# qiyunzhu/woltka

Hardware: AMD Instinct MI355X
Metric: alignment records/sec classified (higher is better)
Workload: dtype u8; 1 GPU; synthetic SAM text of 50M reads x <=16 hits (10.50 GB) resident in HBM, 2M-node taxonomy, ranks phylum,genus,species: device tokenizer per 64 MB block + one weighted histogram per sample (the kernels of `woltka classify`, host link left out); records_per_gpu=250034804, reads_per_gpu=50000000

## Files before the change

### woltka_amd/csrc/wk_dtok_fused.hpp

```cpp
#pragma once
#include "wk_dtok.hpp"
#include "wk_dtok_planes.hpp"
#include "wk_dtok_rounds.hpp"

namespace wk {

constexpr uint32_t kFzThreads = 512;
constexpr uint32_t kFzWaves = kFzThreads / kWave;
constexpr uint32_t kFzTile = 16384;
constexpr uint32_t kFzBack = 1024;
constexpr uint32_t kFzFwd = 3072;
constexpr uint32_t kFzWin = kFzTile + kFzBack + kFzFwd;
constexpr uint32_t kFzChunks = kFzWin / 16 + 1;
constexpr uint32_t kFzRounds = kFrMaxRounds;
static_assert(kFrChunks * 16u == kFzWin && kFrTailChunk + 1u == kFzChunks && kFrWaves == kFzWaves && kFrWave == kWave,
              "the dealing covers the window");
constexpr uint32_t kFzLines = 1024;
constexpr uint32_t kFzStreams = 4;
constexpr uint32_t kFzCap = 1024;
static_assert(kFzCap >= kFzLines, "a window's records fit an empty buffer");
static_assert(kFzWin + 32 < 65536, "window offsets fit 16 bits");
constexpr uint32_t kFzCarry = 256;
static_assert(kFzCarry + kFzLines <= kFpMaxLines && kFzThreads % kWave == 0, "a window's owned lines fit the planes, a wave's lines one word");

constexpr uint32_t kDtokSpill = 64;

struct FusedArgs {
    const unsigned char* text;
    uint32_t n;
    uint32_t open_end;
    uint32_t span;
    const struct DictSlot8* dict8;
    const uint4* names16;
    uint32_t dict_mask;
    const unsigned char* arena;
    uint2* unknown;
    uint32_t unknown_cap;
    DtokState* state;
    DtokState* host_state;
    const unsigned long long* backup_prev;
    unsigned long long* backup_next;
    uint32_t* host_seq;
    uint32_t seq;
    StreamSet streams;
    const int32_t* submap;
    uint32_t n_submap;
    uint32_t ablate;
};

static_assert(sizeof(DtokState) % 8 == 0, "the packed totals are aligned");
__device__ __forceinline__ unsigned long long* fz_totals(DtokState* state) { return reinterpret_cast<unsigned long long*>(state + 1); }

__global__ void dtok_fused_begin_kernel(unsigned long long* __restrict__ backup, const unsigned long long* __restrict__ cursor, DtokState* state) {
    if (threadIdx.x < (uint32_t)kMaxStreams) backup[threadIdx.x] = cursor[threadIdx.x];
    if (threadIdx.x == 0) {
        *state = DtokState{0u, 0u, 0ull, 0ull, 0ull, 0u, 0u};
        *fz_totals(state) = 0ull;
    }
}

template <int kCtrl, int kRowMask>
__device__ __forceinline__ uint32_t fz_dpp_add(uint32_t v) {
    return v + (uint32_t)__builtin_amdgcn_update_dpp(0, (int)v, kCtrl, kRowMask, 0xF, false);
}
__device__ __forceinline__ uint32_t fz_wave_scan(uint32_t v) {
    static_assert(kWave == 64, "four rows of sixteen lanes");
    v = fz_dpp_add<0x111, 0xF>(v);
    v = fz_dpp_add<0x112, 0xF>(v);
    v = fz_dpp_add<0x114, 0xF>(v);
    v = fz_dpp_add<0x118, 0xF>(v);
    v = fz_dpp_add<0x142, 0xA>(v);
    v = fz_dpp_add<0x143, 0xC>(v);
    return v;
}
__device__ __forceinline__ uint32_t fz_last_lane(uint32_t v) { return (uint32_t)__builtin_amdgcn_readlane((int)v, kWave - 1); }
__device__ __forceinline__ uint32_t fz_wave_sum(uint32_t v) { return fz_last_lane(fz_wave_scan(v)); }
__device__ __forceinline__ unsigned long long fz_first_lane64(unsigned long long v) {
    return ((unsigned long long)(uint32_t)__builtin_amdgcn_readfirstlane((int)(uint32_t)(v >> 32)) << 32) |
           (uint32_t)__builtin_amdgcn_readfirstlane((int)(uint32_t)v);
}

__device__ __forceinline__ uint4 fz_load_stream(const unsigned char* p) {
    typedef uint32_t u32x4 __attribute__((ext_vector_type(4)));
    const u32x4 v = __builtin_nontemporal_load(reinterpret_cast<const u32x4*>(p));
    return make_uint4(v.x, v.y, v.z, v.w);
}
__device__ __forceinline__ unsigned long long fz_load64(const unsigned char* p) {
    unsigned long long w;
    __builtin_memcpy(&w, p, 8);
    return w;
}
__device__ __forceinline__ uint32_t fz_load32(const unsigned char* p) {
    uint32_t w;
    __builtin_memcpy(&w, p, 4);
    return w;
}
__device__ __forceinline__ unsigned long long fz_eq_bytes(unsigned long long w, unsigned char c) {
    const unsigned long long x = w ^ (0x0101010101010101ull * c);
    return ~(((x & 0x7F7F7F7F7F7F7F7Full) + 0x7F7F7F7F7F7F7F7Full) | x | 0x7F7F7F7F7F7F7F7Full);
}
__device__ __forceinline__ uint32_t fz_marks32(uint32_t w, uint32_t c4) {
    const uint32_t x = w ^ c4;
    return ~(((x & 0x7F7F7F7Fu) + 0x7F7F7F7Fu) | x | 0x7F7F7F7Fu);
}
__device__ __forceinline__ unsigned long long fz_low_bytes(unsigned long long w, uint32_t k) {
    return k >= 8u ? w : (w & ((1ull << (8u * k)) - 1ull));
}

__device__ __forceinline__ unsigned long long fz_hash(const unsigned char* p, uint32_t n) {
    unsigned long long h = 0xcbf29ce484222325ull ^ ((unsigned long long)n * 0x9E3779B97F4A7C15ull);
    while (n >= 8u) {
        h = (h ^ fz_load64(p)) * 0x100000001b3ull;
        h ^= h >> 29;
        p += 8;
        n -= 8u;
    }
    const unsigned long long v = n ? fz_low_bytes(fz_load64(p), n) : 0ull;
    h = (h ^ v) * 0x100000001b3ull;
    h ^= h >> 32;
    h *= 0x9E3779B97F4A7C15ull;
    return h ^ (h >> 29);
}

__device__ __forceinline__ bool fz_same(const unsigned char* x, const unsigned char* y, uint32_t n) {
    while (n >= 8u) {
        if (fz_load64(x) != fz_load64(y)) return false;
        x += 8;
        y += 8;
        n -= 8u;
    }
    return n == 0u || fz_low_bytes(fz_load64(x) ^ fz_load64(y), n) == 0ull;
}

struct FzProbe {
    unsigned long long hv, n0, n1;
    uint32_t h;
    uint2 slot;
};
__device__ __forceinline__ FzProbe fz_probe_begin(const FusedArgs& a, const unsigned char* name, uint32_t rn) {
    FzProbe p;
    p.hv = fz_hash(name, rn);
    p.n0 = p.n1 = 0ull;
    if (rn <= 15u) {
        p.n0 = fz_low_bytes(fz_load64(name), rn);
        p.n1 = (rn > 8u ? fz_low_bytes(fz_load64(name + 8), rn - 8u) : 0ull) | ((unsigned long long)rn << 56);
    }
    p.h = (uint32_t)p.hv & a.dict_mask;
    p.slot = reinterpret_cast<const uint2*>(a.dict8)[p.h];
    return p;
}
__device__ __forceinline__ int32_t fz_probe_end(const FusedArgs& a, FzProbe p, const unsigned char* name, uint32_t rn, uint32_t abs_off) {
    for (;;) {
        const int32_t id = (int32_t)p.slot.y;
        if (id < 0) break;
        if (p.slot.x == (uint32_t)(p.hv >> 32)) {
            const uint4 nm = a.names16[id];
            const unsigned long long s0 = ((unsigned long long)nm.y << 32) | nm.x, s1 = ((unsigned long long)nm.w << 32) | nm.z;
            if (rn <= 15u) {
                if (s0 == p.n0 && s1 == p.n1) return id;
            } else if ((nm.w >> 24) == 0xFFu) {
                const unsigned char* full = a.arena + nm.x;
                if (fz_load32(full) == rn && fz_same(name, full + 4, rn)) return id;
            }
        }
        p.h = (p.h + 1u) & a.dict_mask;
        p.slot = reinterpret_cast<const uint2*>(a.dict8)[p.h];
    }
    const uint32_t at = atomicAdd(&a.state->n_unknown, 1u);
    if (at < a.unknown_cap)
        a.unknown[at] = make_uint2(abs_off, rn);
    else
        atomicOr(&a.state->flags, kDtokUnknownFull);
    return kLineUnknown;
}

__device__ bool fz_starts_run_slow(const unsigned char* __restrict__ text, uint32_t at, const unsigned char* q, uint32_t qn) {
    uint32_t pos = at;
    while (pos > 0u) {
        const uint32_t e = pos - 1u;
        uint32_t s = e;
        while (s > 0u && text[s - 1u] != '\n') --s;
        uint32_t tab[3], nt = 0;
        for (uint32_t p = s; p < e && nt < 3u; ++p)
            if (text[p] == '\t') tab[nt++] = p;
        if (nt == 3u && !(tab[2] - tab[1] == 2u && text[tab[1] + 1u] == '*')) {
            if (tab[0] - s != qn) return true;
            for (uint32_t k = 0; k < qn; ++k)
                if (text[s + k] != q[k]) return true;
            return false;
        }
        pos = s;
    }
    return true;
}

constexpr uint32_t kFiSubj = (1u << 23) - 1u;
constexpr uint32_t kFiMateShift = 24;
constexpr uint32_t kFiMapped = 1u << 26;
constexpr uint32_t kFiStart = 1u << 27;
constexpr uint32_t kFiExcl = 1u << 29;
constexpr uint32_t kFiDropped = 1u << 30;
constexpr uint32_t kFiRead = kFiMapped | (3u << kFiMateShift);
constexpr uint32_t kFiKey = kFiRead | kFiSubj;
constexpr uint32_t kFzPad = 8;

__device__ __forceinline__ uint32_t fz_octet(uint32_t z_lo, uint32_t z_hi) { return (((z_lo >> 7) | (z_hi >> 3)) * 0x00204081u >> 21) & 255u; }

__device__ __forceinline__ uint32_t fz_newlines16(uint4 v) {
    return fz_octet(fz_marks32(v.x, 0x0A0A0A0Au), fz_marks32(v.y, 0x0A0A0A0Au)) | (fz_octet(fz_marks32(v.z, 0x0A0A0A0Au), fz_marks32(v.w, 0x0A0A0A0Au)) << 8);
}

__device__ __forceinline__ uint32_t fz_tabs32(const unsigned char* p) {
    unsigned long long w[4];
#pragma unroll
    for (uint32_t i = 0; i < 4; ++i) w[i] = fz_load64(p + 8u * i);
    uint32_t m = 0;
#pragma unroll
    for (uint32_t i = 0; i < 4; ++i)
        m |= fz_octet(fz_marks32((uint32_t)w[i], 0x09090909u), fz_marks32((uint32_t)(w[i] >> 32), 0x09090909u)) << (8u * i);
    return m;
}

__global__ void __launch_bounds__(kFzThreads) __attribute__((amdgpu_waves_per_eu(6, 6))) dtok_fused_kernel(FusedArgs a) {
    __shared__ __attribute__((aligned(16))) unsigned char txt[kFzChunks * 16 + 32];
    __shared__ uint16_t ls[kFzLines + 2];
    __shared__ uint16_t f_qn[kFzLines], f_rb[kFzLines], f_rn[kFzLines];
    __shared__ __attribute__((aligned(16))) uint32_t info_[kFzPad + kFzCarry + kFzLines + kFzPad + 8];
    __shared__ uint32_t carry[kFzCarry];
    __shared__ unsigned long long planes[kFpPlanes][kFpWords];
    __shared__ uint32_t rbuf[kFzStreams][kFzCap];
    __shared__ unsigned long long fill_packed;
    static_assert(kFzStreams <= 4 && kFzCap + kFzThreads < 65536, "four 16-bit counts");
    __shared__ unsigned long long gbase[kFzStreams];
    __shared__ uint32_t wtot[kFzWaves];
    __shared__ unsigned long long gbase_out[kMaxStreams];
    __shared__ unsigned long long wg_totals;
    __shared__ uint32_t own[4];
    __shared__ uint32_t wg_flags;
    uint32_t* const info = info_ + kFzPad + kFzCarry;

    const uint32_t tid = threadIdx.x, lane = tid & (kWave - 1), wave = tid / kWave;
    const uint32_t wave_s = (uint32_t)__builtin_amdgcn_readfirstlane((int)wave);
    const uint32_t n_streams = a.streams.n_streams;
    const uint32_t ablate = a.ablate;
    const int32_t* const submap = a.submap;
    unsigned long long fill = 0ull;
    if (tid == 0) fill_packed = 0ull;
    if (tid < 4u) reinterpret_cast<uint32_t*>(txt + kFrTailChunk * 16u)[tid] = 0u;
    if (tid == 0) wg_flags = 0u;
    if (tid == 0) wg_totals = 0ull;
    uint32_t my_flags = 0, my_reads = 0, my_lines = 0;
    const uint32_t text_end = a.n + (a.open_end ? 1u : 0u);

    auto flush_all = [&](unsigned long long have, bool last) {
        __syncthreads();
        if (tid < n_streams) {
            const uint32_t cnt = (ablate & 64u) ? 0u : (uint32_t)(have >> (16u * tid)) & 0xFFFFu;
            unsigned long long base = 0ull;
            if (cnt) {
                base = atomicAdd(&a.streams.cursor[tid], (unsigned long long)cnt);
                if (base + cnt > a.streams.cap) atomicOr(&wg_flags, kDtokSpill);
            }
            gbase[tid] = base;
        }
        __syncthreads();
        for (uint32_t k = 0; k < n_streams; ++k) {
            const uint32_t cnt = (ablate & 64u) ? 0u : (uint32_t)(have >> (16u * k)) & 0xFFFFu;
            const unsigned long long base = gbase[k];
            for (uint32_t i = tid; i < cnt; i += kFzThreads)
                if (base + i < a.streams.cap) a.streams.out[k][base + i] = rbuf[k][i];
        }
        if (last) return;
        __syncthreads();
    };

    const uint32_t t0 = blockIdx.x * a.span;
    const uint32_t t1 = a.n - t0 > a.span ? t0 + a.span : a.n;
    const uint32_t span_w1 = (uint32_t)min((unsigned long long)t1 + kFzFwd, (unsigned long long)text_end);
    uint32_t wpos = t0 >= kFzBack ? t0 - kFzBack : 0u;
    uint32_t mode = 0u;
    uint32_t counted = t0;
    bool wide = false;
    uint32_t nc = 0u;
    uint32_t cq_pos = 0u, cq_len = 0u;
    const uint32_t max_trips = a.span / 16u + 2u;
    for (uint32_t trip = 0;; ++trip) {
        if (trip >= max_trips) {
            my_flags |= kDtokSpill;
            break;
        }
        const uint32_t w0 = wpos & ~15u;
        const uint32_t lead = wpos - w0;
        const uint32_t w1 = (uint32_t)min((mode == 0u ? (unsigned long long)t0 + kFzTile + kFzFwd : (unsigned long long)w0 + kFzWin),
                                           (unsigned long long)(wide ? text_end : span_w1));
        const bool to_end = w1 == text_end;
        const bool last_win = wide || w1 == span_w1;
        __syncthreads();
        if (tid < 3u) own[tid] = tid < 2u ? 0xFFFFFFFFu : 0u;
        if (tid < kFzPad) info[-(int32_t)nc - 1 - (int32_t)tid] = kFiStart;
        for (uint32_t i = tid; i < nc; i += kFzThreads) info[(int32_t)i - (int32_t)nc] = carry[i];

        const uint32_t wave_c0 = fr_first_chunk(wave_s), wave_rounds = fr_rounds(wave_s);
        uint4 v[kFzRounds];
#pragma unroll
        for (uint32_t r = 0; r < kFzRounds; ++r) {
            const uint32_t p = w0 + (wave_c0 + r * kWave + lane) * 16u;
            v[r] = make_uint4(0u, 0u, 0u, 0u);
            if (r < wave_rounds && p < a.n && p < w1) v[r] = fz_load_stream(a.text + p);
        }
        uint32_t marks[kFzRounds];
        uint32_t nl_packed = 0;
        bool blank = false;
        const uint32_t in_lo = max(wpos, counted), in_hi = min(min(w1, a.n), t1);
#pragma unroll
        for (uint32_t r = 0; r < kFzRounds; ++r) {
            const uint32_t c = wave_c0 + r * kWave + lane;
            const uint32_t p = w0 + c * 16u;
            marks[r] = 0u;
            if (r >= wave_rounds) continue;
            const uint32_t rp0 = w0 + (wave_c0 + r * kWave) * 16u;
            const bool interior = rp0 >= in_lo && (unsigned long long)rp0 + kWave * 16u <= in_hi;
            *reinterpret_cast<uint4*>(txt + c * 16u) = v[r];
            if (interior) {
                const uint32_t m = fr_chunk_marks(fz_newlines16(v[r]), &blank);
                const uint32_t cnt = (uint32_t)__popc(m);
                my_lines += cnt;
                marks[r] = m;
                nl_packed |= fr_pack(cnt, r);
            } else if (p < w1) {
                uint32_t m = fz_newlines16(v[r]);
                if (p + 16u > a.n) m &= p >= a.n ? 0u : (1u << (a.n - p)) - 1u;
                if (p >= counted && p < t1) my_lines += (uint32_t)__popc(m);
                if (a.open_end && a.n >= p && a.n < p + 16u) m |= 1u << (a.n - p);
                if (p + 16u > w1) m &= (1u << (w1 - p)) - 1u;
                if (p < wpos) m &= ~((1u << (wpos - p)) - 1u);
                m = fr_chunk_marks(m, &blank);
                marks[r] = m;
                nl_packed |= fr_pack((uint32_t)__popc(m), r);
            }
        }
        if (blank && !(ablate & 16u)) my_flags |= kDtokShortLine;
        const uint32_t nl_inc = fz_wave_scan(nl_packed);
        const uint32_t nl_wave = fz_last_lane(nl_inc);
        if (lane == 0) wtot[wave] = fr_total(nl_wave);
        __syncthreads();
        uint32_t before = 0, total_nl = 0;
#pragma unroll
        for (uint32_t w = 0; w < kFzWaves; ++w) {
            before += w < wave ? wtot[w] : 0u;
            total_nl += wtot[w];
        }
        const bool too_many = total_nl + 1u > kFzLines || (ablate & (32u | 512u));
        if (too_many) {
            if (!(ablate & 512u)) my_flags |= kDtokSpill;
        } else {
            if (tid == 0) ls[0] = (uint16_t)lead;
            uint32_t line = before;
#pragma unroll
            for (uint32_t r = 0; r < kFzRounds; ++r) {
                if (r >= wave_rounds) continue;
                const uint32_t c = wave_c0 + r * kWave + lane;
                uint32_t at = line + fr_unpack(nl_inc, r) - (uint32_t)__popc(marks[r]);
                uint32_t m = marks[r];
                while (m) {
                    const uint32_t b = (uint32_t)__ffs((int)m) - 1u;
                    ls[++at] = (uint16_t)(c * 16u + b + 1u);
                    m &= m - 1u;
                }
                line += fr_unpack(nl_wave, r);
            }
        }
        __syncthreads();
        const uint32_t trail = too_many ? wpos : w0 + (uint32_t)__builtin_amdgcn_readfirstlane((int)(uint32_t)ls[total_nl]);
        if (!too_many && last_win && trail >= t0 && trail < t1) my_flags |= kDtokSpill;
        const uint32_t first_line = mode != 0u || w0 == 0u ? 0u : 1u;
        const uint32_t n_lines = too_many ? 0u : total_nl;
        if (tid == 0 && first_line) info[0] = 0u;

        for (uint32_t k = first_line + tid; k < n_lines; k += kFzThreads) {
            const uint32_t s = ls[k], e = (uint32_t)ls[k + 1] - 1u;
            uint32_t tab[3] = {0, 0, 0}, nt = 0;
            if (!(ablate & 256u)) {
                uint32_t m = fz_tabs32(txt + s);
                if (e - s < 32u) m &= (1u << (e - s)) - 1u;
                nt = min((uint32_t)__popc(m), 3u);
                tab[0] = s + (uint32_t)__ffs((int)m) - 1u;
                m &= m - 1u;
                tab[1] = s + (uint32_t)__ffs((int)m) - 1u;
                m &= m - 1u;
                tab[2] = s + (uint32_t)__ffs((int)m) - 1u;
                for (uint32_t p = s + 32u; nt < 3u && p < e; p += 32u) {
                    m = fz_tabs32(txt + p);
                    if (e - p < 32u) m &= (1u << (e - p)) - 1u;
                    for (; m && nt < 3u; m &= m - 1u) {
                        const uint32_t q = p + (uint32_t)__ffs((int)m) - 1u;
                        if (nt == 0u)
                            tab[0] = q;
                        else if (nt == 1u)
                            tab[1] = q;
                        else
                            tab[2] = q;
                        ++nt;
                    }
                }
            }
            uint32_t word = 0;
            if (ablate & 16u) {
            } else if (nt < 3u) {
                my_flags |= kDtokShortLine;
            } else {
                const uint32_t fl = tab[1] - tab[0] - 1u;
                const unsigned long long fw = fz_load64(txt + tab[0] + 1u);
                uint32_t flag = 0;
                bool digits = fl >= 1u && fl <= 6u;
                for (uint32_t i = 0; i < fl && i < 6u; ++i) {
                    const uint32_t d = ((uint32_t)(fw >> (8u * i)) & 0xFFu) - (uint32_t)'0';
                    digits &= d <= 9u;
                    flag = flag * 10u + d;
                }
                const uint32_t rb = tab[1] + 1u, rn = tab[2] - rb;
                if (!digits) {
                    my_flags |= kDtokShortLine;
                } else if (rn == 1u && txt[rb] == '*') {
                } else {
                    const uint32_t mate = (flag >> 6) & 3u;
                    if (mate == 3u) my_flags |= kDtokBothMates;
                    word = kFiMapped | (mate << kFiMateShift);
                    f_qn[k] = (uint16_t)(tab[0] - s);
                    f_rb[k] = (uint16_t)rb;
                    f_rn[k] = (uint16_t)rn;
                }
            }
            info[k] = word;
        }
        __syncthreads();

        for (uint32_t k = first_line + tid; k < n_lines; k += kFzThreads) {
            if (!(info[k] & kFiMapped) || w0 + ls[k] < t0) continue;
            const unsigned char* name = txt + f_rb[k];
            const uint32_t rn = f_rn[k];
            FzProbe probe;
            if (!(ablate & 1u)) probe = fz_probe_begin(a, name, rn);
            uint32_t j = k;
            bool found = false;
            while (j > first_line) {
                --j;
                if (info[j] & kFiMapped) {
                    found = true;
                    break;
                }
            }
            bool start;
            if (ablate & 8u)
                start = true;
            else if (found)
                start = f_qn[j] != f_qn[k] || !fz_same(txt + ls[k], txt + ls[j], f_qn[k]);
            else if (nc)
                start = f_qn[k] != cq_len || !fz_same(txt + ls[k], a.text + cq_pos, cq_len);
            else if (mode == 1u || wpos == 0u)
                start = true;
            else
                start = fz_starts_run_slow(a.text, w0 + ls[first_line], txt + ls[k], f_qn[k]);
            int32_t sid = (ablate & 1u) ? (int32_t)(fz_load32(name + 4) % 1000u) : fz_probe_end(a, probe, name, rn, w0 + f_rb[k]);
            bool excluded = false;
            if (submap && sid >= 0) {
                if ((uint32_t)sid < a.n_submap) {
                    sid = submap[sid];
                    if (sid == kLineExcluded) {
                        excluded = true;
                        sid = 0;
                    }
                } else {
                    my_flags |= kDtokSpill;
                    sid = -1;
                }
            }
            info[k] |= (start ? kFiStart : 0u) | (excluded ? kFiExcl : 0u) | (sid < 0 ? kFiSubj : ((uint32_t)sid & kFiSubj));
            if (start) {
                atomicMin(&own[w0 + ls[k] < t1 ? 0 : 1], k);
                atomicMax(&own[2], k);
            }
        }
        __syncthreads();
        const uint32_t o0 = (uint32_t)__builtin_amdgcn_readfirstlane((int)own[0]), o1 = (uint32_t)__builtin_amdgcn_readfirstlane((int)own[1]);
        const uint32_t last = (uint32_t)__builtin_amdgcn_readfirstlane((int)own[2]);
        const uint32_t lpos = w0 + (uint32_t)__builtin_amdgcn_readfirstlane((int)(uint32_t)ls[o0 != 0xFFFFFFFFu ? last : 0u]);
        const bool has_first = nc != 0u || o0 != 0xFFFFFFFFu;
        const int32_t first_own = nc ? -(int32_t)nc : (int32_t)o0;
        int32_t ka = 0, kb = 0;
        uint32_t next = 0u, next_mode = 0u, nc_next = 0u;
        bool more = false, again = false, put_aside = false;
        if (too_many) {
            if ((ablate & (32u | 512u)) && !last_win) {
                next = w1;
                next_mode = 2u;
                more = true;
            }
        } else if (o1 != 0xFFFFFFFFu) {
            kb = (int32_t)o1;
            ka = has_first ? first_own : kb;
        } else if (to_end) {
            kb = (int32_t)n_lines;
            ka = has_first ? first_own : kb;
        } else if (last_win && a.span <= kFzTile) {
            if (o0 != 0xFFFFFFFFu) my_flags |= kDtokSpill;
        } else if (o0 != 0xFFFFFFFFu && (nc != 0u || last != o0 || lpos > wpos)) {
            kb = (int32_t)last;
            ka = first_own;
            next = lpos;
            next_mode = 1u;
            more = true;
            again = last_win;
        } else if (o0 != 0xFFFFFFFFu && last_win && !wide) {
            next = wpos;
            next_mode = 1u;
            more = again = true;
        } else if (o0 != 0xFFFFFFFFu || nc != 0u) {
            put_aside = true;
        } else if (!last_win) {
            next = trail;
            next_mode = 2u;
            more = trail > wpos && trail < t1;
            if (trail <= wpos) my_flags |= kDtokSpill;
        }
        if (put_aside) {
            if (tid == 0) {
                uint32_t c = nc;
                for (uint32_t k = first_line; k < n_lines; ++k) {
                    const uint32_t w = info[k];
                    if (w & kFiMapped) {
                        if (c < kFzCarry) carry[c] = w & ~kFiDropped;
                        ++c;
                    }
                }
                own[3] = c;
            }
            __syncthreads();
            nc_next = (uint32_t)__builtin_amdgcn_readfirstlane((int)own[3]);
            if (nc_next > kFzCarry || trail <= wpos) {
                my_flags |= kDtokSpill;
                nc_next = 0u;
            } else {
                if (nc == 0u) {
                    cq_pos = wpos;
                    cq_len = (uint32_t)__builtin_amdgcn_readfirstlane((int)(uint32_t)f_qn[0]);
                }
                next = trail;
                next_mode = 2u;
                more = true;
                again = last_win;
            }
        }
        for (int32_t k0 = ka; k0 < kb; k0 += (int32_t)kFzThreads) {
            const int32_t k = k0 + (int32_t)tid;
            const uint32_t mk = k < kb ? info[k] : 0u;
            const bool mapped = (mk & kFiMapped) != 0u, excl = mapped && (mk & kFiExcl);
            if (excl) {
                int32_t j = k;
                while (!(info[j] & kFiStart)) --j;
                atomicOr(&info[j], kFiDropped);
            }
            bool dup = false;
            if (mapped && !excl && !(mk & kFiStart) && !(ablate & 2u)) {
                bool done = false;
                for (int32_t j = k; !done; j -= 8) {
                    uint32_t w[8];
#pragma unroll
                    for (uint32_t i = 0; i < 8; ++i) w[i] = info[j - 1 - (int32_t)i];
#pragma unroll
                    for (uint32_t i = 0; i < 8; ++i) {
                        dup |= !done && ((w[i] ^ mk) & kFiKey) == 0u;
                        done |= (w[i] & kFiStart) != 0u;
                    }
                }
            }
            const bool first = mapped && !excl && !dup;
            const uint32_t mate = (mk >> kFiMateShift) & 3u;
            const uint32_t wi = (uint32_t)__builtin_amdgcn_readfirstlane((int)((uint32_t)(k0 - ka) / kWave + wave));
            const bool put = lane == 0 && wi < kFpWords;
            const unsigned long long p_start = __ballot(mapped && (mk & kFiStart));
            if (put) planes[kFpStart][wi] = p_start;
#pragma unroll
            for (uint32_t m = 0; m < 4; ++m) {
                const unsigned long long p_first = __ballot(first && mate == m);
                if (put) planes[kFpFirst + m][wi] = p_first;
            }
        }
        __syncthreads();
        for (int32_t k0 = ka; k0 < kb; k0 += (int32_t)kFzThreads) {
            const int32_t k = k0 + (int32_t)tid;
            bool rec = false;
            uint32_t word = 0, sl = 0, at = 0;
            const uint32_t li = (uint32_t)(k - ka);
            const uint32_t mk = k < kb ? info[k] : 0u;
            const unsigned long long* const mine = planes[kFpFirst + ((mk >> kFiMateShift) & 3u)];
            if (k < kb && ((mine[li / 64u] >> (li % 64u)) & 1ull) && !(ablate & 4u)) {
                uint32_t pos = 0, size = 1;
                bool dropped = (mk & kFiStart) && (mk & kFiDropped);
                if (!(ablate & (2u | 128u))) {
                    const FpRead r = fp_read(planes[kFpStart], mine, li, (uint32_t)(kb - ka));
                    pos = r.pos;
                    size = r.size;
                    dropped = (info[ka + (int32_t)r.head] & kFiDropped) != 0u;
                }
                if (size > (uint32_t)WK_WEIGHT_MAX_K) my_flags |= kDtokBigRead;
                const uint32_t s = mk & kFiSubj;
                if (s != kFiSubj && !dropped) {
                    rec = true;
                    word = s | ((pos & 15u) << kWordSubjBits) | ((size & 31u) << kWordSizeShift);
                    sl = s / kSliceBins;
                    if (sl >= n_streams) sl = n_streams - 1u;
                    my_reads += pos == 0u ? 1u : 0u;
                }
            }
            {
                unsigned long long add = 0;
                uint32_t mine_before = 0;
                for (uint32_t s2 = 0; s2 < n_streams; ++s2) {
                    const unsigned long long m = __ballot(rec && sl == s2);
                    add |= (unsigned long long)__popcll(m) << (16u * s2);
                    if (rec && sl == s2) mine_before = (uint32_t)__popcll(m & ((1ull << lane) - 1ull));
                }
                if (add) {
                    unsigned long long base = 0;
                    if (lane == 0) base = atomicAdd(&fill_packed, add);
                    base = fz_first_lane64(base);
                    at = (uint32_t)(base >> (16u * sl)) & 0xFFFFu;
                    at += mine_before;
                }
            }
            __syncthreads();
            unsigned long long now = fz_first_lane64(fill_packed);
            static_assert(kFzCap + 0x7BFFu == 0x7FFFu && 2u * kFzCap + kFzThreads + 0x7BFFu < 0x10000u, "the full test");
            if ((now + 0x7BFF7BFF7BFF7BFFull) & 0x8000800080008000ull) {
                flush_all(fill, false);
                at -= (uint32_t)(fill >> (16u * sl)) & 0xFFFFu;
                now -= fill;
                if (tid == 0) fill_packed = now;
            }
            if (rec) rbuf[sl][at] = word;
            fill = now;
            if (k0 + (int32_t)kFzThreads < kb) __syncthreads();
        }
        if (!more) break;
        wpos = next;
        mode = next_mode;
        wide = again;
        nc = nc_next;
        counted = w1;
    }
    if (my_flags) atomicOr(&wg_flags, my_flags);
    {
        const uint32_t reads_w = fz_wave_sum(my_reads), lines_w = fz_wave_sum(my_lines);
        const unsigned long long t = ((unsigned long long)lines_w << 32) | reads_w;
        if (lane == 0 && t) atomicAdd(&wg_totals, t);
    }
    flush_all(fill, true);
    __syncthreads();
    if (tid == 0) {
        if (wg_totals) __hip_atomic_fetch_add(fz_totals(a.state), wg_totals, __ATOMIC_RELAXED, __HIP_MEMORY_SCOPE_AGENT);
        if (wg_flags) atomicOr(&a.state->flags, wg_flags);
        __threadfence();
        own[0] = atomicAdd(&a.state->done, 1u) == gridDim.x - 1u ? 1u : 0u;
    }
    __syncthreads();
    if (own[0]) {
        __threadfence();
        uint32_t xt = tid;
        asm volatile("" : "+v"(xt));
        if (xt < (uint32_t)kMaxStreams) {
            const unsigned long long cur = __hip_atomic_load(&a.streams.cursor[xt], __ATOMIC_RELAXED, __HIP_MEMORY_SCOPE_AGENT);
            a.backup_next[xt] = cur;
            gbase_out[xt] = xt < n_streams ? cur - a.backup_prev[xt] : 0ull;
        }
        __syncthreads();
        if (tid == 0) {
            DtokState st{};
            st.flags = __hip_atomic_load(&a.state->flags, __ATOMIC_RELAXED, __HIP_MEMORY_SCOPE_AGENT);
            st.n_unknown = __hip_atomic_load(&a.state->n_unknown, __ATOMIC_RELAXED, __HIP_MEMORY_SCOPE_AGENT);
            const unsigned long long totals = __hip_atomic_load(fz_totals(a.state), __ATOMIC_RELAXED, __HIP_MEMORY_SCOPE_AGENT);
            for (uint32_t k = 0; k < (uint32_t)kMaxStreams; ++k) st.n_out += gbase_out[k];
            st.n_reads = totals & 0xFFFFFFFFull;
            st.n_lines = totals >> 32;
            *a.host_state = st;
            *a.state = DtokState{0u, 0u, 0ull, 0ull, 0ull, 0u, 0u};
            *fz_totals(a.state) = 0ull;
            __threadfence_system();
            if (a.host_seq) __hip_atomic_store(a.host_seq, a.seq, __ATOMIC_RELEASE, __HIP_MEMORY_SCOPE_SYSTEM);
        }
    }
}

}
```

Measured before the change: 15.61 billion records/s.

## Fuse line parse and probe passes, decide run starts via DPP neighbour compare

Merges the tab-parsing loop and the lookup/run-start loop into a single pass. The previous line's query-name prefix now comes from a DPP lane shift instead of a backward scan plus byte compare, and only undecided lines (wave edges, unmapped neighbours, long names) fall back to the old scan in a second pass. It also adds a specialised hash for short reference names, batches the own[] atomics through wave ballots, and drops the f_rb/f_rn shared arrays. The cost is extra shared edge buffers, a second loop over all lines, and more register pressure from carrying the parsed fields.

```diff
diff --git a/woltka_amd/csrc/wk_dtok_fused.hpp b/woltka_amd/csrc/wk_dtok_fused.hpp
--- a/woltka_amd/csrc/wk_dtok_fused.hpp
+++ b/woltka_amd/csrc/wk_dtok_fused.hpp
@@ -1,5 +1,6 @@
 #pragma once
 #include "wk_dtok.hpp"
+#include "wk_dtok_neighbour.hpp"
 #include "wk_dtok_planes.hpp"
 #include "wk_dtok_rounds.hpp"
 
@@ -139,11 +140,23 @@
 };
 __device__ __forceinline__ FzProbe fz_probe_begin(const FusedArgs& a, const unsigned char* name, uint32_t rn) {
     FzProbe p;
-    p.hv = fz_hash(name, rn);
     p.n0 = p.n1 = 0ull;
     if (rn <= 15u) {
-        p.n0 = fz_low_bytes(fz_load64(name), rn);
-        p.n1 = (rn > 8u ? fz_low_bytes(fz_load64(name + 8), rn - 8u) : 0ull) | ((unsigned long long)rn << 56);
+        const unsigned long long lo = fz_low_bytes(fz_load64(name), rn), hi = rn > 8u ? fz_low_bytes(fz_load64(name + 8), rn - 8u) : 0ull;
+        p.n0 = lo;
+        p.n1 = hi | ((unsigned long long)rn << 56);
+        unsigned long long h = 0xcbf29ce484222325ull ^ ((unsigned long long)rn * 0x9E3779B97F4A7C15ull), v = lo;
+        if (rn >= 8u) {
+            h = (h ^ lo) * 0x100000001b3ull;
+            h ^= h >> 29;
+            v = hi;
+        }
+        h = (h ^ v) * 0x100000001b3ull;
+        h ^= h >> 32;
+        h *= 0x9E3779B97F4A7C15ull;
+        p.hv = h ^ (h >> 29);
+    } else {
+        p.hv = fz_hash(name, rn);
     }
     p.h = (uint32_t)p.hv & a.dict_mask;
     p.slot = reinterpret_cast<const uint2*>(a.dict8)[p.h];
@@ -198,11 +211,13 @@
 constexpr uint32_t kFiMateShift = 24;
 constexpr uint32_t kFiMapped = 1u << 26;
 constexpr uint32_t kFiStart = 1u << 27;
+constexpr uint32_t kFiUndecided = 1u << 28;
 constexpr uint32_t kFiExcl = 1u << 29;
 constexpr uint32_t kFiDropped = 1u << 30;
 constexpr uint32_t kFiRead = kFiMapped | (3u << kFiMateShift);
 constexpr uint32_t kFiKey = kFiRead | kFiSubj;
 constexpr uint32_t kFzPad = 8;
+constexpr uint32_t kFzEdgeMeta = 4;
 
 __device__ __forceinline__ uint32_t fz_octet(uint32_t z_lo, uint32_t z_hi) { return (((z_lo >> 7) | (z_hi >> 3)) * 0x00204081u >> 21) & 255u; }
 
@@ -210,7 +225,7 @@
     return fz_octet(fz_marks32(v.x, 0x0A0A0A0Au), fz_marks32(v.y, 0x0A0A0A0Au)) | (fz_octet(fz_marks32(v.z, 0x0A0A0A0Au), fz_marks32(v.w, 0x0A0A0A0Au)) << 8);
 }
 
-__device__ __forceinline__ uint32_t fz_tabs32(const unsigned char* p) {
+__device__ __forceinline__ uint32_t fz_tabs32(const unsigned char* p, unsigned long long* q0 = nullptr, unsigned long long* q1 = nullptr) {
     unsigned long long w[4];
 #pragma unroll
     for (uint32_t i = 0; i < 4; ++i) w[i] = fz_load64(p + 8u * i);
@@ -218,13 +233,18 @@
 #pragma unroll
     for (uint32_t i = 0; i < 4; ++i)
         m |= fz_octet(fz_marks32((uint32_t)w[i], 0x09090909u), fz_marks32((uint32_t)(w[i] >> 32), 0x09090909u)) << (8u * i);
+    if (q0) {
+        *q0 = w[0];
+        *q1 = w[1];
+    }
     return m;
 }
 
 __global__ void __launch_bounds__(kFzThreads) __attribute__((amdgpu_waves_per_eu(6, 6))) dtok_fused_kernel(FusedArgs a) {
     __shared__ __attribute__((aligned(16))) unsigned char txt[kFzChunks * 16 + 32];
     __shared__ uint16_t ls[kFzLines + 2];
-    __shared__ uint16_t f_qn[kFzLines], f_rb[kFzLines], f_rn[kFzLines];
+    __shared__ uint16_t f_qn[kFzLines];
+    __shared__ __attribute__((aligned(16))) uint32_t edge[kFzLines / kWave + 1][2][8];
     __shared__ __attribute__((aligned(16))) uint32_t info_[kFzPad + kFzCarry + kFzLines + kFzPad + 8];
     __shared__ uint32_t carry[kFzCarry];
     __shared__ unsigned long long planes[kFpPlanes][kFpWords];
@@ -249,6 +269,7 @@
     if (tid < 4u) reinterpret_cast<uint32_t*>(txt + kFrTailChunk * 16u)[tid] = 0u;
     if (tid == 0) wg_flags = 0u;
     if (tid == 0) wg_totals = 0ull;
+    if (tid == 0) edge[0][1][kFzEdgeMeta] = 0u;
     uint32_t my_flags = 0, my_reads = 0, my_lines = 0;
     const uint32_t text_end = a.n + (a.open_end ? 1u : 0u);
 
@@ -377,108 +398,158 @@
         const uint32_t n_lines = too_many ? 0u : total_nl;
         if (tid == 0 && first_line) info[0] = 0u;
 
-        for (uint32_t k = first_line + tid; k < n_lines; k += kFzThreads) {
-            const uint32_t s = ls[k], e = (uint32_t)ls[k + 1] - 1u;
-            uint32_t tab[3] = {0, 0, 0}, nt = 0;
-            if (!(ablate & 256u)) {
-                uint32_t m = fz_tabs32(txt + s);
-                if (e - s < 32u) m &= (1u << (e - s)) - 1u;
-                nt = min((uint32_t)__popc(m), 3u);
-                tab[0] = s + (uint32_t)__ffs((int)m) - 1u;
-                m &= m - 1u;
-                tab[1] = s + (uint32_t)__ffs((int)m) - 1u;
-                m &= m - 1u;
-                tab[2] = s + (uint32_t)__ffs((int)m) - 1u;
-                for (uint32_t p = s + 32u; nt < 3u && p < e; p += 32u) {
-                    m = fz_tabs32(txt + p);
-                    if (e - p < 32u) m &= (1u << (e - p)) - 1u;
-                    for (; m && nt < 3u; m &= m - 1u) {
-                        const uint32_t q = p + (uint32_t)__ffs((int)m) - 1u;
-                        if (nt == 0u)
-                            tab[0] = q;
-                        else if (nt == 1u)
-                            tab[1] = q;
-                        else
-                            tab[2] = q;
-                        ++nt;
+        for (uint32_t k0 = first_line; k0 < n_lines; k0 += kFzThreads) {
+            const uint32_t k = k0 + tid;
+            const bool has = k < n_lines;
+            uint32_t word = 0, s = 0, qn = 0, rb = 0, rn = 0;
+            unsigned long long q0 = 0ull, q1 = 0ull;
+            if (has) {
+                s = ls[k];
+                const uint32_t e = (uint32_t)ls[k + 1] - 1u;
+                uint32_t tab[3] = {0, 0, 0}, nt = 0;
+                if (!(ablate & 256u)) {
+                    uint32_t m = fz_tabs32(txt + s, &q0, &q1);
+                    if (e - s < 32u) m &= (1u << (e - s)) - 1u;
+                    nt = min((uint32_t)__popc(m), 3u);
+                    tab[0] = s + (uint32_t)__ffs((int)m) - 1u;
+                    m &= m - 1u;
+                    tab[1] = s + (uint32_t)__ffs((int)m) - 1u;
+                    m &= m - 1u;
+                    tab[2] = s + (uint32_t)__ffs((int)m) - 1u;
+                    for (uint32_t p = s + 32u; nt < 3u && p < e; p += 32u) {
+                        m = fz_tabs32(txt + p);
+                        if (e - p < 32u) m &= (1u << (e - p)) - 1u;
+                        for (; m && nt < 3u; m &= m - 1u) {
+                            const uint32_t q = p + (uint32_t)__ffs((int)m) - 1u;
+                            if (nt == 0u)
+                                tab[0] = q;
+                            else if (nt == 1u)
+                                tab[1] = q;
+                            else
+                                tab[2] = q;
+                            ++nt;
+                        }
                     }
                 }
-            }
-            uint32_t word = 0;
-            if (ablate & 16u) {
-            } else if (nt < 3u) {
-                my_flags |= kDtokShortLine;
-            } else {
-                const uint32_t fl = tab[1] - tab[0] - 1u;
-                const unsigned long long fw = fz_load64(txt + tab[0] + 1u);
-                uint32_t flag = 0;
-                bool digits = fl >= 1u && fl <= 6u;
-                for (uint32_t i = 0; i < fl && i < 6u; ++i) {
-                    const uint32_t d = ((uint32_t)(fw >> (8u * i)) & 0xFFu) - (uint32_t)'0';
-                    digits &= d <= 9u;
-                    flag = flag * 10u + d;
-                }
-                const uint32_t rb = tab[1] + 1u, rn = tab[2] - rb;
-                if (!digits) {
+                if (ablate & 16u) {
+                } else if (nt < 3u) {
                     my_flags |= kDtokShortLine;
-                } else if (rn == 1u && txt[rb] == '*') {
                 } else {
-                    const uint32_t mate = (flag >> 6) & 3u;
-                    if (mate == 3u) my_flags |= kDtokBothMates;
-                    word = kFiMapped | (mate << kFiMateShift);
-                    f_qn[k] = (uint16_t)(tab[0] - s);
-                    f_rb[k] = (uint16_t)rb;
-                    f_rn[k] = (uint16_t)rn;
-                }
-            }
-            info[k] = word;
-        }
-        __syncthreads();
-
-        for (uint32_t k = first_line + tid; k < n_lines; k += kFzThreads) {
-            if (!(info[k] & kFiMapped) || w0 + ls[k] < t0) continue;
-            const unsigned char* name = txt + f_rb[k];
-            const uint32_t rn = f_rn[k];
+                    const uint32_t fl = tab[1] - tab[0] - 1u;
+                    const unsigned long long fw = fz_load64(txt + tab[0] + 1u);
+                    uint32_t flag = 0;
+                    bool digits = fl >= 1u && fl <= 6u;
+                    for (uint32_t i = 0; i < fl && i < 6u; ++i) {
+                        const uint32_t d = ((uint32_t)(fw >> (8u * i)) & 0xFFu) - (uint32_t)'0';
+                        digits &= d <= 9u;
+                        flag = flag * 10u + d;
+                    }
+                    rb = tab[1] + 1u;
+                    rn = tab[2] - rb;
+                    if (!digits) {
+                        my_flags |= kDtokShortLine;
+                    } else if (rn == 1u && txt[rb] == '*') {
+                    } else {
+                        const uint32_t mate = (flag >> 6) & 3u;
+                        if (mate == 3u) my_flags |= kDtokBothMates;
+                        word = kFiMapped | (mate << kFiMateShift);
+                        qn = tab[0] - s;
+                        f_qn[k] = (uint16_t)qn;
+                    }
+                }
+            }
+            const bool mapped = (word & kFiMapped) != 0u, look = mapped && w0 + s >= t0;
+            const unsigned char* const name = txt + rb;
             FzProbe probe;
-            if (!(ablate & 1u)) probe = fz_probe_begin(a, name, rn);
-            uint32_t j = k;
-            bool found = false;
-            while (j > first_line) {
-                --j;
-                if (info[j] & kFiMapped) {
-                    found = true;
-                    break;
-                }
-            }
-            bool start;
-            if (ablate & 8u)
-                start = true;
-            else if (found)
-                start = f_qn[j] != f_qn[k] || !fz_same(txt + ls[k], txt + ls[j], f_qn[k]);
-            else if (nc)
-                start = f_qn[k] != cq_len || !fz_same(txt + ls[k], a.text + cq_pos, cq_len);
-            else if (mode == 1u || wpos == 0u)
-                start = true;
-            else
-                start = fz_starts_run_slow(a.text, w0 + ls[first_line], txt + ls[k], f_qn[k]);
-            int32_t sid = (ablate & 1u) ? (int32_t)(fz_load32(name + 4) % 1000u) : fz_probe_end(a, probe, name, rn, w0 + f_rb[k]);
-            bool excluded = false;
-            if (submap && sid >= 0) {
-                if ((uint32_t)sid < a.n_submap) {
-                    sid = submap[sid];
-                    if (sid == kLineExcluded) {
-                        excluded = true;
-                        sid = 0;
+            if (look && !(ablate & 1u)) probe = fz_probe_begin(a, name, rn);
+            const FnLine me = has ? fn_line(mapped, qn, q0, q1) : fn_no_line();
+            FnLine prev;
+            prev.meta = (uint32_t)__builtin_amdgcn_update_dpp(0, (int)me.meta, 0x138 , 0xF, 0xF, false);
+#pragma unroll
+            for (uint32_t i = 0; i < 4; ++i) prev.b[i] = (uint32_t)__builtin_amdgcn_update_dpp(0, (int)me.b[i], 0x138, 0xF, 0xF, false);
+            const uint32_t verdict = (ablate & 8u) ? (uint32_t)kFnStarts : (uint32_t)fn_verdict(prev, me);
+            if (lane == 0 || lane == kWave - 1u) {
+                uint32_t* const to = lane == 0 ? edge[(k0 - first_line) / kWave + wave][0] : edge[(k0 - first_line) / kWave + wave + 1u][1];
+                *reinterpret_cast<uint4*>(to) = make_uint4(me.b[0], me.b[1], me.b[2], me.b[3]);
+                to[kFzEdgeMeta] = me.meta;
+            }
+            const bool start = look && verdict == kFnStarts;
+            if (look) {
+                int32_t sid = (ablate & 1u) ? (int32_t)(fz_load32(name + 4) % 1000u) : fz_probe_end(a, probe, name, rn, w0 + rb);
+                bool excluded = false;
+                if (submap && sid >= 0) {
+                    if ((uint32_t)sid < a.n_submap) {
+                        sid = submap[sid];
+                        if (sid == kLineExcluded) {
+                            excluded = true;
+                            sid = 0;
+                        }
+                    } else {
+                        my_flags |= kDtokSpill;
+                        sid = -1;
                     }
-                } else {
-                    my_flags |= kDtokSpill;
-                    sid = -1;
-                }
-            }
-            info[k] |= (start ? kFiStart : 0u) | (excluded ? kFiExcl : 0u) | (sid < 0 ? kFiSubj : ((uint32_t)sid & kFiSubj));
-            if (start) {
-                atomicMin(&own[w0 + ls[k] < t1 ? 0 : 1], k);
-                atomicMax(&own[2], k);
+                }
+                word |= (start ? kFiStart : 0u) | (verdict == kFnUndecided ? kFiUndecided : 0u) | (excluded ? kFiExcl : 0u) |
+                        (sid < 0 ? kFiSubj : ((uint32_t)sid & kFiSubj));
+            }
+            if (has) info[k] = word;
+            const unsigned long long b_all = __ballot(start), b_in = __ballot(start && w0 + s < t1), b_out = b_all & ~b_in;
+            if (lane == 0 && b_all) {
+                if (b_in) atomicMin(&own[0], k + (uint32_t)__builtin_ctzll(b_in));
+                if (b_out) atomicMin(&own[1], k + (uint32_t)__builtin_ctzll(b_out));
+                atomicMax(&own[2], k + 63u - (uint32_t)__builtin_clzll(b_all));
+            }
+        }
+        __syncthreads();
+        for (uint32_t k0 = first_line; k0 < n_lines; k0 += kFzThreads) {
+            const uint32_t k = k0 + tid;
+            const uint32_t mk = k < n_lines ? info[k] : 0u;
+            bool und = (mk & kFiUndecided) != 0u, start = false;
+            if (lane == 0 && und) {
+                const uint32_t g = (k0 - first_line) / kWave + wave;
+                FnLine before, me;
+#pragma unroll
+                for (uint32_t i = 0; i < 4; ++i) {
+                    before.b[i] = edge[g][1][i];
+                    me.b[i] = edge[g][0][i];
+                }
+                before.meta = edge[g][1][kFzEdgeMeta];
+                me.meta = edge[g][0][kFzEdgeMeta];
+                const FnVerdict v = fn_verdict(before, me);
+                und = v == kFnUndecided;
+                start = v == kFnStarts;
+                if (g == 0u && nc == 0u && (mode == 1u || wpos == 0u)) {
+                    und = false;
+                    start = true;
+                }
+            }
+            if (__ballot(und) != 0ull) {
+                if (und) {
+                    uint32_t j = k;
+                    bool found = false;
+                    while (j > first_line) {
+                        --j;
+                        if (info[j] & kFiMapped) {
+                            found = true;
+                            break;
+                        }
+                    }
+                    if (found)
+                        start = f_qn[j] != f_qn[k] || !fz_same(txt + ls[k], txt + ls[j], f_qn[k]);
+                    else if (nc)
+                        start = f_qn[k] != cq_len || !fz_same(txt + ls[k], a.text + cq_pos, cq_len);
+                    else if (mode == 1u || wpos == 0u)
+                        start = true;
+                    else
+                        start = fz_starts_run_slow(a.text, w0 + ls[first_line], txt + ls[k], f_qn[k]);
+                }
+            }
+            if (mk & kFiUndecided) {
+                info[k] = (mk & ~kFiUndecided) | (start ? kFiStart : 0u);
+                if (start) {
+                    atomicMin(&own[w0 + ls[k] < t1 ? 0 : 1], k);
+                    atomicMax(&own[2], k);
+                }
             }
         }
         __syncthreads();
diff --git a/woltka_amd/csrc/wk_dtok_neighbour.hpp b/woltka_amd/csrc/wk_dtok_neighbour.hpp
--- /dev/null
+++ b/woltka_amd/csrc/wk_dtok_neighbour.hpp
@@ -0,0 +1,45 @@
+#pragma once
+#include <cstdint>
+
+#if defined(__HIPCC__) || defined(__CUDACC__)
+#define WK_FN_FN __host__ __device__ __forceinline__
+#else
+#define WK_FN_FN inline
+#endif
+
+namespace wk {
+
+constexpr uint32_t kFnLine = 1u << 16;
+constexpr uint32_t kFnMapped = 1u << 17;
+constexpr uint32_t kFnQn = 0xFFFFu;
+constexpr uint32_t kFnBytes = 16;
+
+struct FnLine {
+    uint32_t meta;
+    uint32_t b[4];
+};
+
+enum FnVerdict : uint32_t { kFnStarts = 0, kFnContinues = 1, kFnUndecided = 2 };
+
+WK_FN_FN unsigned long long fn_low_bytes(unsigned long long w, uint32_t k) { return k >= 8u ? w : (w & ((1ull << (8u * k)) - 1ull)); }
+
+WK_FN_FN FnLine fn_line(bool mapped, uint32_t qn, unsigned long long w0, unsigned long long w1) {
+    FnLine l;
+    l.meta = kFnLine | (mapped ? kFnMapped : 0u) | (qn & kFnQn);
+    const unsigned long long m0 = fn_low_bytes(w0, qn), m1 = qn > 8u ? fn_low_bytes(w1, qn - 8u) : 0ull;
+    l.b[0] = (uint32_t)m0;
+    l.b[1] = (uint32_t)(m0 >> 32);
+    l.b[2] = (uint32_t)m1;
+    l.b[3] = (uint32_t)(m1 >> 32);
+    return l;
+}
+WK_FN_FN FnLine fn_no_line() { return FnLine{0u, {0u, 0u, 0u, 0u}}; }
+
+WK_FN_FN FnVerdict fn_verdict(const FnLine& prev, const FnLine& cur) {
+    if ((prev.meta & (kFnLine | kFnMapped)) != (kFnLine | kFnMapped)) return kFnUndecided;
+    const uint32_t diff = ((prev.meta ^ cur.meta) & kFnQn) | (prev.b[0] ^ cur.b[0]) | (prev.b[1] ^ cur.b[1]) | (prev.b[2] ^ cur.b[2]) | (prev.b[3] ^ cur.b[3]);
+    if (diff) return kFnStarts;
+    return (cur.meta & kFnQn) <= kFnBytes ? kFnContinues : kFnUndecided;
+}
+
+}
```

Measured after the change: 16.21 billion records/s (median of 6 runs). +3.8%, better.
